# wienkers/marEx

Measured on AMD Instinct MI355X. Metric: Mcells*timesteps/s, shifting_baseline + hobday_extreme p95 (validation+anomaly+thresholds+mask), higher is better.
Workload: dtype f32

## Files before the change

marex_amd/csrc/marex_shifting.hip:

```cpp
#include "marex_common.hip.h"
#include "marex_tails.hip.h"
#include <numeric>
#include <utility>

template <int D, int SCAP, bool SEXACT, int WCAP, bool RREG>
__global__ void __launch_bounds__(256)
k_shifting(const float* __restrict__ x, long T, long C, const int4* __restrict__ year_plan, int n_cal, int W,
           int S_rt, int write_clim, const float* __restrict__ edges, int nb, long T_out, float* __restrict__ out,
           unsigned short* __restrict__ bins, unsigned char* __restrict__ mask, int* __restrict__ invalid_count,
           int ncb, int nchunks, const int* __restrict__ skip) {
    extern __shared__ float lds[];
    float* ring = lds;
    float rr[RREG ? D : 1][RREG ? WCAP : 1];
    const int npad = WCAP - W;
    int4* lplan = reinterpret_cast<int4*>(lds + (RREG ? (size_t)0 : (size_t)D * WCAP * 256));
    float* e = reinterpret_cast<float*>(lplan + (size_t)n_cal * D);

    int cb, chunk;
    if (!xcd_swizzle(blockIdx.x, ncb, nchunks, cb, chunk)) return;
    if (D == 4 && skip && skip[chunk]) return;
    const int tid = threadIdx.x;
    const long c = (long)cb * 256 + tid;
    const bool active = c < C;
    const int S = SEXACT ? SCAP : S_rt;
// ... 343 lines not shown
            int4 e[4];
            for (int i = 0; i < 4; ++i)
                e[i] = (d0 + i < NDOY) ? year_plan[(size_t)y * NDOY + d0 + i] : make_int4(-1, -1, -1, 0);
            int m = 0;
            while (m < 4 && e[m].x >= 0) ++m;
            if (fplan) {
                const int yn = y + 1 < n_cal ? y + 1 : n_cal - 1;
                const int tbw = year_plan[(size_t)yn * NDOY + (chunk >> 2) * 16].x;
                fplan[((size_t)y * 92 + chunk) * 2] = make_int4(e[0].x, e[0].y, m, e[0].z);
                fplan[((size_t)y * 92 + chunk) * 2 + 1] = make_int4(e[1].z, e[2].z, e[3].z, tbw);
            }
            for (int i = m; i < 4; ++i) ok = ok && e[i].x < 0;
            for (int i = 1; i < m; ++i) {
                ok = ok && e[i].x == e[0].x + i;
                if (e[0].y >= 0)
                    ok = ok && e[i].y == e[0].y + i && e[i].z >= 0;
                else
                    ok = ok && e[i].y < 0;
            }
            if (m > 0 && e[0].y >= 0) ok = ok && e[0].z >= 0;
        }
        if (!ok) atomicAnd(&s_ok[chunk], 0);
    }
    __syncthreads();
    if (chunk < 92 && lplan && reg_S > 0) {
        const int H = reg_S / 2, NPAIR = (reg_S + 3) / 2, NROWS = wpb * ((reg_S + 4 * wpb - 1 + wpb - 1) / wpb);
        const int d0 = chunk * 4, blk16 = (chunk / wpb) * wpb * 4;
        int D1 = 0, D2 = 0, D3 = 0;
        if (lean_bins && d0 + 3 < NDOY)
            for (int y2 = 0; y2 < n_cal; ++y2) {
                const int z0 = year_plan[(size_t)y2 * NDOY + d0].z, z1 = year_plan[(size_t)y2 * NDOY + d0 + 1].z;
                const int z2 = year_plan[(size_t)y2 * NDOY + d0 + 2].z, z3 = year_plan[(size_t)y2 * NDOY + d0 + 3].z;
                if (z0 >= 0 && z1 >= 0 && z2 >= 0 && z3 >= 0) {
                    D1 = z1 - z0;
                    D2 = z2 - z0;
                    D3 = z3 - z0;
                    break;
                }
            }
        for (int yy = sub - 1; yy <= n_cal; yy += CLASSIFY_SPLIT) {
            int flags = 0, tbv = -1, pos = 0;
            long long xoff = 0, ooff = 0;
            if (yy + 1 >= 0 && yy + 1 < n_cal) {
                const int tbn = year_plan[(size_t)(yy + 1) * NDOY + blk16].x;
                if (tbn >= H && (long)tbn - H + NROWS <= T) {
                    flags |= 4;
                    xoff = (long long)(tbn - H) * C * 4;
                }
            }
            if (yy >= 0 && yy < n_cal) {
                int4 e[4];
                for (int i = 0; i < 4; ++i) e[i] = (d0 + i < NDOY) ? year_plan[(size_t)yy * NDOY + d0 + i] : make_int4(-1, -1, -1, 0);
                tbv = year_plan[(size_t)yy * NDOY + blk16].x;
                int reg = d0 + 3 < NDOY && e[0].x >= 0 && e[1].x >= 0 && e[2].x >= 0 && e[3].x >= 0;
                reg = reg && tbv >= H && (long)tbv - H + NROWS <= T && e[0].x == tbv + 4 * (chunk % wpb);
                reg = reg && e[0].x - H >= 0 && (long)e[0].x - H + 2 * NPAIR <= T;
                for (int i = 1; i < 4; ++i) reg = reg && e[i].x == e[0].x + i && ((e[0].y >= 0) == (e[i].y >= 0));
                if (e[0].y >= 0) {
                    flags |= 2;
                    ooff = (long long)e[0].y * C * 4;
                    if (lean_bins) {
                        pos = e[0].z;
                        reg = reg && pos >= 0 && e[1].z == pos + D1 && e[2].z == pos + D2 && e[3].z == pos + D3;
                        for (int i = 1; i < 4; ++i) reg = reg && e[i].y == e[0].y + i;
                    } else {
                        pos = e[0].z - doy_start[d0];
                        reg = reg && pos >= 0 && pos < TAIL_MAX_BUCKET;
                        for (int i = 1; i < 4; ++i) reg = reg && e[i].y == e[0].y + i && e[i].z - doy_start[d0 + i] == pos;
                    }
                }
                if (reg) flags |= 1;
            }
            int4* r = lplan + ((size_t)(yy + 1) * LEAN_CHUNKS + chunk) * 2;
            r[0] = make_int4(flags, tbv, (int)(unsigned)(xoff & 0xFFFFFFFFll), (int)(unsigned)((unsigned long long)xoff >> 32));
            r[1] = make_int4((int)(unsigned)(ooff & 0xFFFFFFFFll), (int)(unsigned)((unsigned long long)ooff >> 32), pos, 0);
            if (yy < 0 && lean_bins) r[1] = make_int4(0, D1, D2, D3);
            if (chunk + 4 >= 92 && chunk + 4 < (92 + wpb - 1) / wpb * wpb) {
                r[8] = make_int4(flags & 4, tbv, (int)(unsigned)(xoff & 0xFFFFFFFFll), (int)(unsigned)((unsigned long long)xoff >> 32));
                r[9] = make_int4(0, 0, 0, 0);
            }
        }
    }
    if (t < 92) info[t] = s_ok[t] && s_edges_ok;
}

#define SHIFT_LIST 15
struct TailOut {
    uint4* lists;
    unsigned* aux;
    const int* doy_start;
    int nper;
    unsigned long long* dbg;
};

template <int W, bool TAILS, int S = 21>
__global__ void __launch_bounds__(256)
k_shift_fast(const float* __restrict__ x, long T, long C, const int4* __restrict__ fplan, int n_cal,
             const int* __restrict__ info, int write_clim, const float* __restrict__ edges, int nb, long T_out, float* __restrict__ out, unsigned short* __restrict__ bins, unsigned char* __restrict__ mask,
             int* __restrict__ invalid_count, int ncg, int nblk, TailOut tails) {
    int cg, bc;
    if (!xcd_swizzle(blockIdx.x, ncg, nblk, cg, bc)) return;
    const int wave = __builtin_amdgcn_readfirstlane((int)(threadIdx.x >> 6));
    const int lane = (int)(threadIdx.x & 63);
    const int chunk = bc * 4 + wave;
    static_assert((S & 1) == 1 && S >= 5 && S <= 25, "k_shift_fast: odd smoothing widths 5..25");
    constexpr int H = S / 2, NPAIR = (S + 3) / 2, NST = S + 15, RPW = (NST + 3) / 4;
    constexpr int NSTAGE = TAILS ? 1 : 2;
    constexpr int NROWS = NST;
    __shared__ float stage[NSTAGE][NROWS * 64];
    __shared__ unsigned newkeys[TAILS ? 4 : 1][2][TAILS ? SHIFT_LIST : 1][64];
    const bool mine = chunk < 92 && info[chunk] != 0;
    const int d0 = mine ? chunk * 4 : 0;
    const int4* prec = fplan + (size_t)chunk * 2;
    constexpr size_t YREC = 92 * 2;
    const long c = (long)cg * 64 + lane;
    const bool active = c < C;
    const unsigned cidx = active ? (unsigned)c : (unsigned)(C - 1);
    const bool do_bins = bins != nullptr && !TAILS;
    const unsigned voff = cidx * 4u;
    const int rowb = (int)(C * 4);
    const unsigned bin_lane = (((cidx >> 4) - (unsigned)(cg * 4)) * (unsigned)T_out * 16u + (cidx & 15u)) * 2u;
    const rsrc_t rbins = make_rsrc(do_bins ? bins + (size_t)(cg * 4) * (size_t)T_out * 16 : nullptr);

    float e_first = 0.f, e_delta = 1.f, inv_width = 1.f, e_last = 0.f;
    if (do_bins || TAILS) {
        e_first = edges[1];
        e_delta = edges[2] - edges[1];
        e_last = edges[nb];
        inv_width = (float)(nb - 1) / (e_last - e_first);
    }
    constexpr float Sf = (float)S;
    const float yS = 1.0f / Sf;
    const float Wf = (float)W;
    const float yW = 1.0f / Wf;
    const float nbm1f = (float)(nb - 1);
    const float c0 = (1.0f - e_first * inv_width) - 0.0078125f;
    const float qnan = nan_f();

    if (chunk == 0 && mine && mask && active) mask[c] = finite_f(x[c]) ? 1 : 0;
    auto stage_ok = [&](int tb) { return tb >= H && (long)tb - H + NROWS <= T; };
    auto stage_load = [&](int tb, float (&nx)[RPW]) {
        const rsrc_t rs = make_rsrc(x + (size_t)(tb - H + RPW * wave) * C);
#pragma unroll
        for (int k = 0; k < RPW; ++k)
            if (4 * RPW == NST || RPW * wave + k < NST) nx[k] = ldb_f32(rs, voff, k * rowb);
    };
    auto stage_store = [&](int buf, const float (&nx)[RPW]) {
#pragma unroll
        for (int k = 0; k < RPW; ++k)
            if (4 * RPW == NST || RPW * wave + k < NST) stage[buf & (NSTAGE - 1)][(RPW * wave + k) * 64 + lane] = nx[k];
    };
    int tb_cur = fplan[(size_t)(bc * 4) * 2].x;
    int tb_n1 = prec[1].w;
    {
        float nx[RPW];
        if (stage_ok(tb_cur)) {
            stage_load(tb_cur, nx);
            stage_store(0, nx);
        }
        __syncthreads();
    }

    v2f rA[W + 2], rB[W + 2];
#pragma unroll
    for (int j = 0; j < W + 2; ++j) rA[j] = rB[j] = splat2(qnan);
    int n_invalid = 0;
    unsigned t_cntA = 0, t_cntB = 0, t_ovfA = 0, t_ovfB = 0;
    int t_slot = 0, t_list = 0;
    int t_ds0 = 0, t_ds1 = 0, t_ds2 = 0, t_ds3 = 0;
    if (TAILS && mine) {
        t_ds0 = tails.doy_start[d0];
        t_ds1 = tails.doy_start[d0 + 1 < NDOY ? d0 + 1 : NDOY - 1];
        t_ds2 = tails.doy_start[d0 + 2 < NDOY ? d0 + 2 : NDOY - 1];
        t_ds3 = tails.doy_start[d0 + 3 < NDOY ? d0 + 3 : NDOY - 1];
    }
    auto tails_flush = [&]() {
        const tl_out_rsrc_t rl = tl_out_make_rsrc(tails.lists + (size_t)d0 * tails.nper * 2 * (size_t)C);
        const unsigned lvoff = cidx * 16u;
#pragma unroll
        for (int pr = 0; pr < 2; ++pr) {
            unsigned v[16];
#pragma unroll
            for (int u = 0; u < 16; ++u) v[u] = (u < SHIFT_LIST && u < t_slot) ? newkeys[wave][pr][u][lane] : 0u;
            sort16_desc(v);
#pragma unroll
            for (int h = 0; h < 2; ++h) {
                const int di = 2 * pr + h;
                if (d0 + di < NDOY) {
#pragma unroll
                    for (int jj = 0; jj < 2; ++jj) {
                        unsigned w[4];
#pragma unroll
                        for (int i = 0; i < 4; ++i) {
                            const unsigned a = v[8 * jj + 2 * i], b = v[8 * jj + 2 * i + 1];
                            w[i] = h == 0 ? ((a & 0xFFFFu) | (b << 16)) : ((a >> 16) | (b & 0xFFFF0000u));
                        }
                        const int li = __builtin_amdgcn_readfirstlane((di * tails.nper + t_list) * 2 + jj);
                        tl_out_store(rl, lvoff, (unsigned)li * (unsigned)C * 16u, w);
                    }
                }
            }
        }
        ++t_list;
        t_slot = 0;
    };

    int4 nA = prec[0], nB = prec[1];
    auto one_year = [&](int y, auto Jc) {
        constexpr int J = decltype(Jc)::value;
        const int4 pA = nA, pB = nB;
        const int tb = tb_cur;
        float nx[RPW];
        const bool stage_next = y + 1 < n_cal && stage_ok(tb_n1);
        if (stage_next) stage_load(tb_n1, nx);
        v2f smA = splat2(qnan), smB = splat2(qnan);
        v2f xp[NPAIR];
        const bool staged = mine && pA.z > 0 && stage_ok(tb) && pA.x == tb + 4 * wave;
        if (staged) {
            const float* st = &stage[y & (NSTAGE - 1)][(4 * wave) * 64 + lane];
#pragma unroll
            for (int m = 0; m < NPAIR; ++m) {
                xp[m].x = st[(2 * m) * 64];
                xp[m].y = st[(2 * m + 1) * 64];
            }
        }
        if (TAILS) {
            asm volatile("s_waitcnt lgkmcnt(0)\n\ts_barrier" ::: "memory");
        }
        else asm volatile("" ::: "memory");
        {
            const int y1 = y + 1 < n_cal ? y + 1 : n_cal - 1;
            nA = prec[(size_t)y1 * YREC];
            nB = prec[(size_t)y1 * YREC + 1];
            tb_cur = tb_n1;
            tb_n1 = nB.w;
        }
        if (mine && pA.z > 0) {
            const long r0 = (long)pA.x - H;
            const bool edge = r0 < 0 || r0 + 2 * NPAIR > T;
            if (staged) {
            } else if (!edge) {
                const rsrc_t rx = make_rsrc(x + (size_t)r0 * C);
#pragma unroll
                for (int m = 0; m < NPAIR; ++m) {
                    xp[m].x = ldb_f32(rx, voff, (2 * m) * rowb);
                    xp[m].y = ldb_f32(rx, voff, (2 * m + 1) * rowb);
                }
            } else {
#pragma unroll
                for (int m = 0; m < NPAIR; ++m) {
                    long ra = r0 + 2 * m, rb = ra + 1;
                    ra = ra < 0 ? 0 : (ra > T - 1 ? T - 1 : ra);
                    rb = rb < 0 ? 0 : (rb > T - 1 ? T - 1 : rb);
                    xp[m].x = ldb_f32(make_rsrc(x + (size_t)ra * C), voff, 0);
                    xp[m].y = ldb_f32(make_rsrc(x + (size_t)rb * C), voff, 0);
                }
            }
            v2f accA = (v2f){xp[0].x, -0.0f};
#pragma unroll
// ... 58 lines not shown
                                ++n[i];
                            }
                    }
                    if (!(climA.x == climA.x)) climA.x = acc[0] / (float)n[0];
                    if (!(climA.y == climA.y)) climA.y = acc[1] / (float)n[1];
                    if (!(climB.x == climB.x)) climB.x = acc[2] / (float)n[2];
                    if (!(climB.y == climB.y)) climB.y = acc[3] / (float)n[3];
                }
                const v2f aA = xcA - climA, aB = xcB - climB;
                const rsrc_t ro = make_rsrc(out + (size_t)pA.y * C);
                stb_f32(ro, voff, 0, write_clim ? climA.x : aA.x);
                if (has1) stb_f32(ro, voff, rowb, write_clim ? climA.y : aA.y);
                if (has2) stb_f32(ro, voff, 2 * rowb, write_clim ? climB.x : aB.x);
                if (has3) stb_f32(ro, voff, 3 * rowb, write_clim ? climB.y : aB.y);
                if (do_bins || TAILS) {
                    auto digit2 = [&](v2f a, int& k0, int& k1) {
                        const v2f f = __builtin_elementwise_fma(a, splat2(inv_width), splat2(c0));
                        v2f t;
                        t.x = __builtin_amdgcn_fmed3f(__builtin_floorf(f.x), 0.0f, nbm1f);
                        t.y = __builtin_amdgcn_fmed3f(__builtin_floorf(f.y), 0.0f, nbm1f);
                        const v2f phi = t * splat2(e_delta);
                        const v2f ehi = splat2(e_first) + phi;
                        k0 = (int)t.x + (a.x >= ehi.x ? 1 : 0);
                        k1 = (int)t.y + (a.y >= ehi.y ? 1 : 0);
                        if (!TAILS) {
                            k0 = (a.x == a.x) ? k0 : nb;
                            k1 = (a.y == a.y) ? k1 : nb;
                        }
                    };
                    int k0, k1, k2, k3;
                    digit2(aA, k0, k1);
                    digit2(aB, k2, k3);
                    if (TAILS) {
                        const float l1 = has1 ? e_last : -__builtin_inff(), l2 = has2 ? e_last : -__builtin_inff(),
                                    l3 = has3 ? e_last : -__builtin_inff();
                        const bool v0 = aA.x < e_last, v1 = aA.y < l1, v2 = aB.x < l2, v3 = aB.y < l3;
                        const unsigned b0 = 128u + (unsigned)(pA.w - t_ds0), b1 = 128u + (unsigned)(pB.x - t_ds1);
                        const unsigned b2 = 128u + (unsigned)(pB.y - t_ds2), b3 = 128u + (unsigned)(pB.z - t_ds3);
                        const unsigned q0 = v0 ? ((unsigned)k0 << TAIL_POS_BITS) + b0 : 0u, q1 = v1 ? ((unsigned)k1 << TAIL_POS_BITS) + b1 : 0u;
                        const unsigned q2 = v2 ? ((unsigned)k2 << TAIL_POS_BITS) + b2 : 0u, q3 = v3 ? ((unsigned)k3 << TAIL_POS_BITS) + b3 : 0u;
                        newkeys[wave][0][t_slot][lane] = q0 | (q1 << 16);
                        newkeys[wave][1][t_slot][lane] = q2 | (q3 << 16);
                        t_cntA += (v0 ? 1u : 0u) + (v1 ? 0x10000u : 0u);
                        t_cntB += (v2 ? 1u : 0u) + (v3 ? 0x10000u : 0u);
                        const float mx = fmaxf(fmaxf(aA.x, has1 ? aA.y : aA.x), fmaxf(has2 ? aB.x : aA.x, has3 ? aB.y : aA.x));
                        if (__builtin_amdgcn_ballot_w64(mx >= e_last) != 0) {
                            unsigned s0 = t_ovfA & 0xFFFFu, s1 = t_ovfA >> 16, s2 = t_ovfB & 0xFFFFu, s3 = t_ovfB >> 16;
                            if (aA.x >= e_last) s0 = tail_ovf_add(s0, (unsigned)(pA.w - t_ds0));
                            if (has1 && aA.y >= e_last) s1 = tail_ovf_add(s1, (unsigned)(pB.x - t_ds1));
                            if (has2 && aB.x >= e_last) s2 = tail_ovf_add(s2, (unsigned)(pB.y - t_ds2));
                            if (has3 && aB.y >= e_last) s3 = tail_ovf_add(s3, (unsigned)(pB.z - t_ds3));
                            t_ovfA = s0 | (s1 << 16);
                            t_ovfB = s2 | (s3 << 16);
                        }
                        ++t_slot;
                    } else {
                        stb_u16(rbins, bin_lane, pA.w * 32, k0);
                        if (has1) stb_u16(rbins, bin_lane, pB.x * 32, k1);
                        if (has2) stb_u16(rbins, bin_lane, pB.y * 32, k2);
                        if (has3) stb_u16(rbins, bin_lane, pB.z * 32, k3);
                    }
                }
            }
        }
        rA[J + W] = smA;
        rB[J + W] = smB;
        if (stage_next) stage_store((y + 1) & 1, nx);
        __syncthreads();
    };
    for (int y = 0; y < n_cal; y += 2) {
        one_year(y, std::integral_constant<int, 0>{});
        if (TAILS && t_slot == SHIFT_LIST) tails_flush();
        if (y + 1 < n_cal) one_year(y + 1, std::integral_constant<int, 1>{});
        if (TAILS && t_slot == SHIFT_LIST) tails_flush();
#pragma unroll
        for (int j = 0; j < W; ++j) {
            rA[j] = rA[j + 2];
            rB[j] = rB[j + 2];
        }
    }
    if (TAILS && mine) {
        if (t_slot > 0) tails_flush();
        while (t_list < tails.nper) tails_flush();
        if (active) {
            const unsigned cn[4] = {t_cntA & 0xFFFFu, t_cntA >> 16, t_cntB & 0xFFFFu, t_cntB >> 16};
            const unsigned ov[4] = {t_ovfA & 0xFFFFu, t_ovfA >> 16, t_ovfB & 0xFFFFu, t_ovfB >> 16};
#pragma unroll
            for (int di = 0; di < 4; ++di)
                if (d0 + di < NDOY) tails.aux[(size_t)(d0 + di) * C + c] = tail_aux_word(cn[di], ov[di]);
        }
    }
    if (invalid_count && active && n_invalid) atomicAdd(&invalid_count[c], n_invalid);
}

template <typename F, int... Is>
__device__ __forceinline__ void unroll_steps_impl(F& f, std::integer_sequence<int, Is...>) {
    (f(std::integral_constant<int, Is>{}), ...);
}
template <int N, typename F>
__device__ __forceinline__ void unroll_steps(F&& f) {
    unroll_steps_impl(f, std::make_integer_sequence<int, N>{});
}

#define LR_REG 1
#define LR_OUT 2
#define LR_STAGE_NEXT 4

template <int W, int S, int NWV, bool BINS>
__global__ void __launch_bounds__(64 * NWV, 16 / NWV)
k_shift_lean(const float* __restrict__ x, int T, int C, const int4* __restrict__ fplan, const int4* __restrict__ lplan, int n_cal,
             const int* __restrict__ info, const float* __restrict__ edges, int nb, float* __restrict__ out,
             unsigned char* __restrict__ mask, int* __restrict__ invalid_count, int ncg, int nblk, TailOut tails,
             unsigned short* __restrict__ bins, long T_out) {
    int cg, bc;
    if (!xcd_swizzle(blockIdx.x, ncg, nblk, cg, bc)) return;
    const int wave = __builtin_amdgcn_readfirstlane((int)(threadIdx.x >> 6));
    const int lane = (int)(threadIdx.x & 63);
    const int chunk = bc * NWV + wave;
    static_assert((S & 1) == 1 && S >= 5 && S <= 25, "k_shift_lean: odd smoothing widths 5..25");
    static_assert(NWV == 4 || NWV == 8, "k_shift_lean: 4 or 8 waves");
    constexpr int H = S / 2, NPAIR = (S + 3) / 2, NST = S + 4 * NWV - 1, RPW = (NST + NWV - 1) / NWV;
    constexpr int NROWS = NWV * RPW;
    __shared__ float stage[NROWS * 64];
    __shared__ unsigned newkeys[BINS ? 1 : NWV][2][BINS ? 1 : SHIFT_LIST][64];
    const bool mine = chunk < 92 && info[chunk] != 0;
    const int d0 = mine ? chunk * 4 : 0;
    const int c = cg * 64 + lane;
    const bool active = c < C;
    const unsigned cidx = active ? (unsigned)c : (unsigned)(C - 1);
    const unsigned voff = cidx * 4u;
    const int rowb = C * 4;
    const float e_first = edges[1], e_delta = edges[2] - edges[1], e_last = edges[nb];
    const float inv_width = (float)(nb - 1) / (e_last - e_first);
    constexpr float Sf = (float)S;
    const float yS = 1.0f / Sf;
    const float Wf = (float)W;
    const float yW = 1.0f / Wf;
    const float nbm1f = (float)(nb - 1);
    const float c0 = (1.0f - e_first * inv_width) - 0.0078125f;
    const float qnan = nan_f();
    if (chunk == 0 && mine && mask && active) mask[c] = finite_f(x[c]) ? 1 : 0;
    const unsigned bin_lane = (((cidx >> 4) - (unsigned)(cg * 4)) * (unsigned)T_out * 16u + (cidx & 15u)) * 2u;
    const rsrc_t rbins = make_rsrc(BINS ? bins + (size_t)(cg * 4) * (size_t)T_out * 16 : nullptr);
    int bD1 = 0, bD2 = 0, bD3 = 0;

    typedef __attribute__((address_space(3))) float lds_f32;
    const int c4 = cg * 64 + (lane & 15) * 4;
    const unsigned dma_voff4 = (unsigned)(lane >> 4) * (unsigned)rowb + (unsigned)(c4 + 4 <= C ? c4 : C - 4) * 4u;
    const unsigned dma_lds = (unsigned)__builtin_amdgcn_readfirstlane((int)(unsigned)(size_t)(lds_f32*)&stage[(RPW * wave) * 64]);
    const char* xw = reinterpret_cast<const char*>(x) + (size_t)(RPW * wave) * (size_t)C * 4;
    auto dma_rows = [&](int lo, int hi) __attribute__((always_inline)) {
        const unsigned long long off = ((unsigned long long)(unsigned)hi << 32) | (unsigned)lo;
        DmaRows<RPW>::issue(tl_out_make_rsrc(xw + off), dma_voff4, voff, dma_lds, 256u, 0u, (unsigned)rowb);
    };
    constexpr int LSTRIDE = LEAN_CHUNKS * 2;
    const int4* lr_next = lplan + (size_t)chunk * 2;
    {
        const int4 pre = lr_next[0];
        if (BINS) {
            const int4 preB = lr_next[1];
            bD1 = preB.y;
            bD2 = preB.z;
            bD3 = preB.w;
        }
        if (pre.x & LR_STAGE_NEXT) {
            dma_rows(pre.z, pre.w);
            asm volatile("s_waitcnt vmcnt(0)" ::: "memory");
        }
        asm volatile("s_barrier" ::: "memory");
        lr_next += LSTRIDE;
    }
    int4 nA = lr_next[0], nB = lr_next[1];
    lr_next += LSTRIDE;

    constexpr int U = W >= 13 ? 3 : 2;
    v2f hA[W + U], hB[W + U];
#pragma unroll
    for (int j = 0; j < W + U; ++j) hA[j] = hB[j] = splat2(qnan);
    int n_invalid = 0;
    unsigned t_cntA = 0, t_cntB = 0, t_ovfA = 0, t_ovfB = 0;
    int t_slot = 0, t_list = 0;
    auto tails_flush = [&]() __attribute__((always_inline)) {
        const tl_out_rsrc_t rl = tl_out_make_rsrc(tails.lists + (size_t)d0 * tails.nper * 2 * (size_t)C);
        const unsigned lvoff = cidx * 16u;
#pragma unroll
        for (int pr = 0; pr < 2; ++pr) {
            unsigned v[16];
#pragma unroll
            for (int u = 0; u < 16; ++u) v[u] = (u < SHIFT_LIST && u < t_slot) ? newkeys[wave][pr][u][lane] : 0u;
            sort16_desc(v);
#pragma unroll
            for (int h = 0; h < 2; ++h) {
                const int di = 2 * pr + h;
                if (d0 + di < NDOY) {
#pragma unroll
                    for (int jj = 0; jj < 2; ++jj) {
                        unsigned w[4];
#pragma unroll
                        for (int i = 0; i < 4; ++i) {
                            const unsigned a = v[8 * jj + 2 * i], b = v[8 * jj + 2 * i + 1];
                            w[i] = h == 0 ? ((a & 0xFFFFu) | (b << 16)) : ((a >> 16) | (b & 0xFFFF0000u));
                        }
                        const int li = __builtin_amdgcn_readfirstlane((di * tails.nper + t_list) * 2 + jj);
                        if (active) tl_out_store(rl, lvoff, (unsigned)li * (unsigned)C * 16u, w);
                    }
                }
            }
        }
        ++t_list;
        t_slot = 0;
    };

    auto mid = [&](const int4& cA) __attribute__((always_inline)) {
        asm volatile("s_waitcnt lgkmcnt(0)\n\ts_barrier" ::: "memory");
        if (cA.x & LR_STAGE_NEXT) dma_rows(cA.z, cA.w);
        nA = lr_next[0];
        nB = lr_next[1];
        lr_next += LSTRIDE;
    };
    constexpr int NH0 = (NPAIR + 1) / 2, NH1 = NPAIR - NH0;
    static_assert(NH0 >= 2, "the second chain starts in the first half");
    v2f xh[NH0];
    v2f accA = splat2(0.f), accB = splat2(0.f);
    float xc0 = 0.f, xc1 = 0.f, xc2 = 0.f, xc3 = 0.f;
    auto load_half = [&](auto Pc, int how, int ts) __attribute__((always_inline)) {
        constexpr int P = decltype(Pc)::value, M0 = P ? NH0 : 0, MN = P ? NH1 : NH0;
        if (how == 0) {
            const float* st = &stage[(4 * wave) * 64 + lane];
#pragma unroll
            for (int m = 0; m < MN; ++m) {
                xh[m].x = st[(2 * (M0 + m)) * 64];
                xh[m].y = st[(2 * (M0 + m) + 1) * 64];
            }
        } else if (how == 1) {
            const rsrc_t rx = make_rsrc(x + (size_t)(ts - H) * (size_t)C);
#pragma unroll
            for (int m = 0; m < MN; ++m) {
                xh[m].x = ldb_f32(rx, voff, (2 * (M0 + m)) * rowb);
                xh[m].y = ldb_f32(rx, voff, (2 * (M0 + m) + 1) * rowb);
            }
        } else {
#pragma unroll
            for (int m = 0; m < MN; ++m) {
                int ra = ts - H + 2 * (M0 + m), rb = ra + 1;
                ra = ra < 0 ? 0 : (ra > T - 1 ? T - 1 : ra);
                rb = rb < 0 ? 0 : (rb > T - 1 ? T - 1 : rb);
                xh[m].x = ldb_f32(make_rsrc(x + (size_t)ra * (size_t)C), voff, 0);
                xh[m].y = ldb_f32(make_rsrc(x + (size_t)rb * (size_t)C), voff, 0);
            }
        }
    };
    auto half = [&](auto Pc) __attribute__((always_inline)) {
        constexpr int P = decltype(Pc)::value, M0 = P ? NH0 : 0, M1 = P ? NPAIR : NH0;
        if constexpr (S == 21) {
#define PK_LO(acc, src) "v_pk_add_f32 %" #acc ", %" #acc ", %" #src " op_sel_hi:[1,0]\n\t"
#define PK_HI(acc, src) "v_pk_add_f32 %" #acc ", %" #acc ", %" #src " op_sel:[0,1] op_sel_hi:[1,1]\n\t"
#define PK_BOTH(src) PK_LO(0, src) PK_LO(1, src) PK_HI(0, src) PK_HI(1, src)
            if (P == 0) {
                accA = (v2f){xh[0].x, -0.0f};
                accB = (v2f){xh[1].x, -0.0f};
                asm(PK_HI(0, 2) PK_LO(0, 3) PK_HI(0, 3) PK_HI(1, 3) PK_BOTH(4) PK_BOTH(5) PK_BOTH(6) PK_BOTH(7)
                    : "+v"(accA), "+v"(accB)
                    : "v"(xh[0]), "v"(xh[1]), "v"(xh[2]), "v"(xh[3]), "v"(xh[4]), "v"(xh[5]));
                xc0 = xh[5].x;
                xc1 = xh[5].y;
// ... 211 lines not shown
            if (has2) n_invalid += finite_f(xcB.x) ? 0 : 1; else smB.x = qnan;
            if (has3) n_invalid += finite_f(xcB.y) ? 0 : 1; else smB.y = qnan;
            asm volatile("s_waitcnt vmcnt(0)" ::: "memory");
            if (pA.y >= 0) {
                v2f aA, aB;
                anomaly(Jc, xcA, xcB, aA, aB);
                const rsrc_t ro = make_rsrc(out + (size_t)pA.y * (size_t)C);
                if (active) {
                    stb_f32(ro, voff, 0, aA.x);
                    if (has1) stb_f32(ro, voff, rowb, aA.y);
                    if (has2) stb_f32(ro, voff, 2 * rowb, aB.x);
                    if (has3) stb_f32(ro, voff, 3 * rowb, aB.y);
                }
                int k0, k1, k2, k3;
                digit2(aA, k0, k1);
                digit2(aB, k2, k3);
                if constexpr (BINS) {
                    if (active) {
                        stb_u16(rbins, bin_lane, pA.w * 32, (aA.x == aA.x) ? k0 : nb);
                        if (has1) stb_u16(rbins, bin_lane, pB.x * 32, (aA.y == aA.y) ? k1 : nb);
                        if (has2) stb_u16(rbins, bin_lane, pB.y * 32, (aB.x == aB.x) ? k2 : nb);
                        if (has3) stb_u16(rbins, bin_lane, pB.z * 32, (aB.y == aB.y) ? k3 : nb);
                    }
                } else {
                const float l1 = has1 ? e_last : -__builtin_inff(), l2 = has2 ? e_last : -__builtin_inff(),
                            l3 = has3 ? e_last : -__builtin_inff();
                const bool v0 = aA.x < e_last, v1 = aA.y < l1, v2 = aB.x < l2, v3 = aB.y < l3;
                const int ds0 = tails.doy_start[d0], ds1 = tails.doy_start[d0 + 1 < NDOY ? d0 + 1 : NDOY - 1];
                const int ds2 = tails.doy_start[d0 + 2 < NDOY ? d0 + 2 : NDOY - 1], ds3 = tails.doy_start[d0 + 3 < NDOY ? d0 + 3 : NDOY - 1];
                const unsigned p0 = (unsigned)(pA.w - ds0), p1 = (unsigned)(pB.x - ds1), p2 = (unsigned)(pB.y - ds2), p3 = (unsigned)(pB.z - ds3);
                const unsigned q0 = v0 ? ((unsigned)k0 << TAIL_POS_BITS) + 128u + p0 : 0u, q1 = v1 ? ((unsigned)k1 << TAIL_POS_BITS) + 128u + p1 : 0u;
                const unsigned q2 = v2 ? ((unsigned)k2 << TAIL_POS_BITS) + 128u + p2 : 0u, q3 = v3 ? ((unsigned)k3 << TAIL_POS_BITS) + 128u + p3 : 0u;
                newkeys[wave][0][t_slot][lane] = q0 | (q1 << 16);
                newkeys[wave][1][t_slot][lane] = q2 | (q3 << 16);
                t_cntA += (v0 ? 1u : 0u) + (v1 ? 0x10000u : 0u);
                t_cntB += (v2 ? 1u : 0u) + (v3 ? 0x10000u : 0u);
                const float mx = fmaxf(fmaxf(aA.x, has1 ? aA.y : aA.x), fmaxf(has2 ? aB.x : aA.x, has3 ? aB.y : aA.x));
                if (__builtin_amdgcn_ballot_w64(mx >= e_last) != 0) {
                    unsigned s0 = t_ovfA & 0xFFFFu, s1 = t_ovfA >> 16, s2 = t_ovfB & 0xFFFFu, s3 = t_ovfB >> 16;
                    if (aA.x >= e_last) s0 = tail_ovf_add(s0, p0);
                    if (has1 && aA.y >= e_last) s1 = tail_ovf_add(s1, p1);
                    if (has2 && aB.x >= e_last) s2 = tail_ovf_add(s2, p2);
                    if (has3 && aB.y >= e_last) s3 = tail_ovf_add(s3, p3);
                    t_ovfA = s0 | (s1 << 16);
                    t_ovfB = s2 | (s3 << 16);
                }
                ++t_slot;
                }
            }
        } else {
            mid(cA);
            asm volatile("s_waitcnt vmcnt(0)" ::: "memory");
        }
        hA[J + W] = smA;
        hB[J + W] = smB;
    };

#define MAREX_LEAN_YEAR(J, yy)                                                                                  \
    {                                                                                                           \
        const int4 cA = nA, cB = nB;                                                                            \
        if (mine && (cA.x & LR_REG)) {                                                                          \
            lean_year(std::integral_constant<int, J>{}, cA, cB);                                                \
        } else {                                                                                                \
            general_year(std::integral_constant<int, J>{}, yy, cA);                                             \
        }                                                                                                       \
        asm volatile("s_barrier" ::: "memory");  \
        if (!BINS && t_slot == SHIFT_LIST) tails_flush();                                                       \
    }
    for (int y = 0; y < n_cal; y += U) {
        MAREX_LEAN_YEAR(0, y)
        if constexpr (U > 1) if (y + 1 < n_cal) MAREX_LEAN_YEAR(1, y + 1)
        if constexpr (U > 2) if (y + 2 < n_cal) MAREX_LEAN_YEAR(2, y + 2)
        if constexpr (U > 3) if (y + 3 < n_cal) MAREX_LEAN_YEAR(3, y + 3)
#pragma unroll
        for (int j = 0; j < W; ++j) {
            hA[j] = hA[j + U];
            hB[j] = hB[j + U];
        }
    }
#undef MAREX_LEAN_YEAR
    if (mine && !BINS) {
        if (t_slot > 0) tails_flush();
        while (t_list < tails.nper) tails_flush();
        if (active) {
            const unsigned cn[4] = {t_cntA & 0xFFFFu, t_cntA >> 16, t_cntB & 0xFFFFu, t_cntB >> 16};
            const unsigned ov[4] = {t_ovfA & 0xFFFFu, t_ovfA >> 16, t_ovfB & 0xFFFFu, t_ovfB >> 16};
#pragma unroll
            for (int di = 0; di < 4; ++di)
                if (d0 + di < NDOY) tails.aux[(size_t)(d0 + di) * (size_t)C + c] = tail_aux_word(cn[di], ov[di]);
        }
    }
    if (invalid_count && active && n_invalid) atomicAdd(&invalid_count[c], n_invalid);
}

static bool lean_instance(int W, int S) { return S == 21 && (W == 15 || W == 5); }

struct ShiftArgs {
    const float* x;
    int64_t T, C;
    const int4* year_plan;
    const int4* fplan;
    int n_cal;
    int W, S, write_clim;
    const float* edges;
    int nb;
    int64_t T_out;
    float* out;
    uint16_t* bins;
    uint8_t* mask;
    int32_t* invalid_count;
    const int* skip;
    TailOut tails;
    bool lean = false;
    const int4* lplan = nullptr;
    int lean_waves = 4;
};

template <int D, int SCAP, bool SEXACT, int WCAP, bool RREG>
static int launch_shifting(marex_ctx* ctx, const ShiftArgs& a) {
    const int ncb = (int)((a.C + 255) / 256);
    const int nchunks = (NDOY + D - 1) / D;
    const size_t lds = ((RREG ? (size_t)0 : (size_t)D * WCAP * 256) + (a.bins ? (size_t)a.nb + 1 : 0)) * sizeof(float) + (size_t)a.n_cal * D * 16;
    if (lds > 80 * 1024) return fail(ctx, -4, "marex_shifting_baseline_f32: window_year_baseline=%d needs more than 80 KiB of LDS", a.W);
    auto kern = k_shifting<D, SCAP, SEXACT, WCAP, RREG>;
    if (lds > 48 * 1024)
        HIP_TRY(ctx, hipFuncSetAttribute((const void*)kern, hipFuncAttributeMaxDynamicSharedMemorySize, (int)lds));
    hipLaunchKernelGGL(kern, dim3(xcd_grid(ncb, nchunks)), dim3(256), lds, ctx->stream, a.x, (long)a.T, (long)a.C,
                       a.year_plan, a.n_cal, a.W, a.S, a.write_clim, a.edges, a.nb, (long)a.T_out, a.out, a.bins,
                       a.mask, a.invalid_count, ncb, nchunks, D == 4 ? a.skip : nullptr);
    HIP_TRY(ctx, hipGetLastError());
    return 0;
}

template <int W, int S = 21>
static void launch_shift_fast(marex_ctx* ctx, const ShiftArgs& a) {
    const int ncg = (int)((a.C + 63) / 64);
#define MAREX_SF_ARGS dim3(xcd_grid(ncg, 23)), dim3(256), 0, ctx->stream, a.x, (long)a.T, (long)a.C, a.fplan, a.n_cal, a.skip, a.write_clim, a.edges, a.nb, (long)a.T_out, a.out, a.bins, a.mask, a.invalid_count, ncg, 23, a.tails
    if (a.lean && (a.tails.lists || a.bins)) {
        if constexpr (S == 21 && (W == 15 || W == 5)) {
            if (a.tails.lists)
                hipLaunchKernelGGL((k_shift_lean<W, S, 4, false>), dim3(xcd_grid(ncg, 23)), dim3(256), 0, ctx->stream, a.x, (int)a.T, (int)a.C,
                                   a.fplan, a.lplan, a.n_cal, a.skip, a.edges, a.nb, a.out, a.mask, a.invalid_count, ncg, 23, a.tails,
                                   (unsigned short*)nullptr, (long)a.T_out);
            else
                hipLaunchKernelGGL((k_shift_lean<W, S, 4, true>), dim3(xcd_grid(ncg, 23)), dim3(256), 0, ctx->stream, a.x, (int)a.T, (int)a.C,
                                   a.fplan, a.lplan, a.n_cal, a.skip, a.edges, a.nb, a.out, a.mask, a.invalid_count, ncg, 23, a.tails,
                                   a.bins, (long)a.T_out);
        }
    } else if (a.tails.lists) {
        hipLaunchKernelGGL((k_shift_fast<W, true, S>), MAREX_SF_ARGS);
    } else {
        hipLaunchKernelGGL((k_shift_fast<W, false, S>), MAREX_SF_ARGS);
    }
#undef MAREX_SF_ARGS
}

template <int D, int WCAP, bool RREG>
static int dispatch_shifting_S(marex_ctx* ctx, const ShiftArgs& a) {
    if (a.S == 21) return launch_shifting<D, 21, true, WCAP, RREG>(ctx, a);
    return launch_shifting<D, 1, false, WCAP, RREG>(ctx, a);
}

static int shifting_impl(marex_ctx* ctx, const char* who, const float* x, int64_t T, int64_t C, const int32_t* year_plan,
                         int n_cal_years, int W, int S, int write_clim, const float* edges, int nb, int64_t T_out, float* out,
                         uint16_t* bins, uint8_t* mask, int32_t* invalid_count, TailOut tails, bool* all_fast_possible) {
    if (!ctx) return -1;
    if (!x || !year_plan || !out || T <= 0 || C <= 0 || n_cal_years <= 0)
        return fail(ctx, -1, "%s: null pointer or empty shape", who);
// ... 116 lines not shown
```

marex_amd/csrc/marex_tails.hip:

```cpp
#include "marex_common.hip.h"
#include "marex_tails.hip.h"

typedef __amdgpu_buffer_rsrc_t tl_rsrc_t;
__device__ __forceinline__ tl_rsrc_t tl_make_rsrc(const void* base) {
    return __builtin_amdgcn_make_buffer_rsrc(const_cast<void*>(base), 0, -1, 0x00020000);
}
__device__ __forceinline__ uint4 tl_load_chunk(tl_rsrc_t r, unsigned voff, unsigned soff) {
    typedef unsigned u4 __attribute__((ext_vector_type(4)));
    const u4 v = __builtin_amdgcn_raw_buffer_load_b128(r, (int)voff, (int)soff, 0);
    return make_uint4(v.x, v.y, v.z, v.w);
}
__device__ __forceinline__ unsigned pk_sub_sat_u16(unsigned a, unsigned b) {
    unsigned r;
    asm("v_pk_sub_u16 %0, %1, %2 clamp" : "=v"(r) : "v"(a), "v"(b));
    return r;
}
__device__ __forceinline__ unsigned pk_add_u16(unsigned a, unsigned b) {
    unsigned r;
    asm("v_pk_add_u16 %0, %1, %2" : "=v"(r) : "v"(a), "v"(b));
    return r;
}
__device__ __forceinline__ unsigned pk_sub_u16(unsigned a, unsigned b) {
    unsigned r;
    asm("v_pk_sub_u16 %0, %1, %2" : "=v"(r) : "v"(a), "v"(b));
// ... 746 lines not shown
            if (pass >= pass_limit) {
                if (!resolved) {
                    thr[(size_t)d * C + cell] = nan_f();
                    atomicAdd(&stats->n_unresolved, 1u);
                }
                break;
            }
            if (lo) {
                B0 = clamp_base(tried_lo - TT_STEP);
                tried_lo = B0;
            } else {
                B0 = clamp_base(tried_hi + TT_STEP);
                tried_hi = B0;
            }
            BW = nb - B0 < TT_BW ? nb - B0 : TT_BW;
            excursion = true;
            rebuild(d);
            tot_s[ci] = prefix();
            hint = -1;
            ++n_pass;
        }
        if (dd + 1 < ndays) {
            const int imin = s_iumin[dpar], imax = s_iumax[dpar];
            if (imax >= 0) {
                const int span = imax - imin + 1;
                const bool near_edge = imin - B0 < TT_MARGIN || (B0 + BW - 1) - imax < TT_MARGIN;
                if (excursion || near_edge) {
                    const int want = clamp_base(span <= TT_BW - 2 * TT_MARGIN ? imin - (TT_BW - span) / 2 : imin - TT_MARGIN);
                    if (want != B0) {
                        B0 = want;
                        BW = nb - B0 < TT_BW ? nb - B0 : TT_BW;
                        need_rebuild = true;
                    }
                }
            }
        }
    }
    for (int sft = 32; sft > 0; sft >>= 1) {
        const unsigned a = __shfl_down(kmin, sft, 64), b = __shfl_down(kmax, sft, 64);
        kmin = a < kmin ? a : kmin;
        kmax = b > kmax ? b : kmax;
        nlow += __shfl_down(nlow, sft, 64);
        nhigh += __shfl_down(nhigh, sft, 64);
    }
    if ((t & 63) == 0) {
        if (kmin != 0xFFFFFFFFu) atomicMin(&stats->min_key, kmin);
        if (kmax != 0u) atomicMax(&stats->max_key, kmax);
        if (nlow) atomicAdd(&stats->n_too_low, nlow);
        if (nhigh) atomicAdd(&stats->n_too_high, nhigh);
    }
    if (dbg && t == 0) {
        atomicAdd(&dbg[0], n_rebuild);
        atomicAdd(&dbg[2], n_pass);
        atomicAdd(&dbg[3], (unsigned long long)ndays);
    }
}

template <int NSC>
__global__ void __launch_bounds__(64)
k_thr_cells(const uint4* __restrict__ lists, const unsigned* __restrict__ aux, int NPER, int nch, const float* __restrict__ anom,
            long C, long c0, long c1, int nblk, const float* __restrict__ centres, int nb, double q, int wd, float lower_bound,
            float upper_bound, float* __restrict__ thr, marex_thr_stats* __restrict__ stats, unsigned long long* __restrict__ dbg) {
    extern __shared__ uint4 ring[];
    const int lane = (int)threadIdx.x;
    const long cell_raw = c0 + (long)blockIdx.x * 64 + lane;
    const bool valid = cell_raw < c1;
    const long cell = valid ? cell_raw : c1 - 1;
    const int d_begin = (int)blockIdx.y * NDOY / nblk, d_end = ((int)blockIdx.y + 1) * NDOY / nblk;
    const bool land = !(anom[cell] == anom[cell]);
    if (__builtin_amdgcn_ballot_w64(valid && !land) == 0) {
        if (valid)
            for (int d = d_begin; d < d_end; ++d) thr[(size_t)d * C + cell] = nan_f();
        return;
    }
    const int pd = wd / 2, nslot = (wd * NPER + 3) & ~3;
    uint4* mine = ring + lane;
    for (int k = wd * NPER; k < nslot; ++k) mine[k * 64] = make_uint4(0, 0, 0, 0);
    const unsigned voff = (unsigned)cell * 16u, chunk_row = (unsigned)C * 16u;
    const size_t day_stride = (size_t)NPER * nch * (size_t)C;
    auto wrap = [](int d) { return d < 0 ? d + NDOY : (d >= NDOY ? d - NDOY : d); };
    auto cnt_of = [&](int day) { return (int)(aux[(size_t)day * C + cell] & 0x3FFu); };
    auto load_day = [&](int day, int k) {
        const tl_rsrc_t r = tl_make_rsrc(lists + (size_t)day * day_stride);
        for (int p = 0; p < NPER; ++p) mine[((k % wd) * NPER + p) * 64] = tl_load_chunk(r, voff, (unsigned)(nch * p) * chunk_row);
    };
    int tot = 0;
    for (int o = 0; o < wd; ++o) {
        const int day = wrap(d_begin - pd + o);
        load_day(day, o);
        tot += cnt_of(day);
    }
    uint4 cache[NSC > 0 ? NSC : 1];
    auto count_ring = [&](int b) {
        const unsigned lim = ((unsigned)(b + 1) << TAIL_POS_BITS) - 1u, lim_rep = lim | (lim << 16);
        unsigned acc0 = 0, acc1 = 0;
        if (NSC > 0) {
#pragma unroll
            for (int k = 0; k < NSC; ++k) {
                acc0 += pk_min1_u16(pk_sub_sat_u16(cache[k].x, lim_rep)) + pk_min1_u16(pk_sub_sat_u16(cache[k].z, lim_rep));
                acc1 += pk_min1_u16(pk_sub_sat_u16(cache[k].y, lim_rep)) + pk_min1_u16(pk_sub_sat_u16(cache[k].w, lim_rep));
            }
        } else
        for (int k = 0; k < nslot; k += 4) {
            const uint4 c[4] = {mine[k * 64], mine[(k + 1) * 64], mine[(k + 2) * 64], mine[(k + 3) * 64]};
#pragma unroll
            for (int u = 0; u < 4; ++u) {
                acc0 += pk_min1_u16(pk_sub_sat_u16(c[u].x, lim_rep)) + pk_min1_u16(pk_sub_sat_u16(c[u].z, lim_rep));
                acc1 += pk_min1_u16(pk_sub_sat_u16(c[u].y, lim_rep)) + pk_min1_u16(pk_sub_sat_u16(c[u].w, lim_rep));
            }
        }
        const unsigned acc = acc0 + acc1;
        return (int)((acc & 0xFFFFu) + (acc >> 16));
    };
    auto count_exact = [&](int d, int b) {
        const unsigned lim = ((unsigned)(b + 1) << TAIL_POS_BITS) - 1u, lim_rep = lim | (lim << 16);
        int n = 0;
        for (int o = -pd; o <= pd; ++o) {
            const tl_rsrc_t r = tl_make_rsrc(lists + (size_t)wrap(d + o) * day_stride);
            for (int p = 0; p < NPER; ++p)
                for (int jj = 0; jj < nch; ++jj) n += tl_count_above(tl_load_chunk(r, voff, (unsigned)(nch * p + jj) * chunk_row), lim_rep);
        }
        return n;
    };
    unsigned kmin = 0xFFFFFFFFu, kmax = 0u, nlow = 0u, nhigh = 0u;
    unsigned long long n_exact = 0;
    for (int d = d_begin; d < d_end; ++d) {
        if (d > d_begin) {
            const int din = wrap(d + pd), dout = wrap(d - pd - 1);
            load_day(din, d - d_begin - 1);
            tot += cnt_of(din) - cnt_of(dout);
        }
        if (NSC > 0) {
#pragma unroll
            for (int k = 0; k < NSC; ++k) cache[k] = mine[k * 64];
        }
        unsigned kfull = 0, khead = 0, ktail = 0xFFFFu;
        int nlists = 0;
        for (int k = 0; k < nslot; k += 4) {
            const uint4 c[4] = {mine[k * 64], mine[(k + 1) * 64], mine[(k + 2) * 64], mine[(k + 3) * 64]};
#pragma unroll
            for (int u = 0; u < 4; ++u) {
                kfull = c[u].w > kfull ? c[u].w : kfull;
                const unsigned head = c[u].x & 0xFFFFu;
                khead = head > khead ? head : khead;
                ktail = (head != 0u && head < ktail) ? head : ktail;
                nlists += head != 0u ? 1 : 0;
            }
        }
        kfull >>= 16;
        float t32 = nan_f();
        if (tot > 0) {
            const double qpos = q * (double)tot;
            int lo = -1, hi = nb - 1, n_lo = tot, n_hi = 0;
            if (khead != 0u && (double)tot > qpos) {
                const int bh = (int)(khead >> TAIL_POS_BITS) - 1;
                hi = bh < hi ? bh : hi;
            }
            bool lo_exact = true;
            if (nlists > 0 && (double)(tot - nlists) <= qpos) {
                const int bt = (int)(ktail >> TAIL_POS_BITS) - 2;
                if (bt > lo && bt < hi) {
                    lo = bt;
                    n_lo = nlists;
                    lo_exact = false;
                }
            }
            while (__builtin_amdgcn_ballot_w64(hi - lo > 1) != 0) {
                const bool go = hi - lo > 1;
                const int mid = go ? (lo + hi) >> 1 : hi;
                int n = count_ring(mid + 1);
                const unsigned first = (unsigned)(mid + 2) << TAIL_POS_BITS;
                bool exact = !(first <= kfull);
                bool f = (double)(tot - n) <= qpos;
                if (__builtin_amdgcn_ballot_w64(go && !f && !exact) != 0) {
                    const int ne = count_exact(d, mid + 1);
                    if (go && !f && !exact) {
                        n = ne;
                        exact = true;
                        f = (double)(tot - n) <= qpos;
                        ++n_exact;
                    }
                }
                if (go) {
                    if (f) {
                        lo = mid;
                        n_lo = n;
                        lo_exact = exact;
                    } else {
                        hi = mid;
                        n_hi = n;
                    }
                }
            }
            const int iu = hi;
            if (__builtin_amdgcn_ballot_w64(iu > 0 && !lo_exact) != 0) {
                const int ne = count_exact(d, iu);
                if (iu > 0 && !lo_exact) {
                    n_lo = ne;
                    ++n_exact;
                }
            }
            const int il = iu > 0 ? iu - 1 : 0;
            const int cs_iu = tot - n_hi, cs_il = iu > 0 ? tot - n_lo : cs_iu;
            const int diff = cs_iu - cs_il;
            const double frac = diff > 0 ? (qpos - (double)cs_il) / (double)diff : 0.5;
            const float dc = centres[iu] - centres[il];
            const double prod = frac * (double)dc;
            t32 = (float)((double)centres[il] + prod);
            if (iu == 0) t32 = centres[0];
            if (valid && !land) {
                const unsigned key = ordered_key(t32);
                kmin = key < kmin ? key : kmin;
                kmax = key > kmax ? key : kmax;
// ... 96 lines not shown
            const long cost = ((blocks + slots - 1) / slots) * (d + wd);
            if (best < 0 || cost < best) best = cost, Dd = d;
        }
    }
    dim3 grid((unsigned)(tiles_x * tiles_y), (unsigned)((NDOY + Dd - 1) / Dd));
    unsigned long long* dbg = ctx_debug_counters(ctx);
    const uint4* tl = reinterpret_cast<const uint4*>(lists);
    const int pass_limit = ctx_opt(ctx, "THR_PASS_LIMIT", 2 * (nb / TT_STEP) + 9);
#define MAREX_TT_ARGS tl, aux, NPER, nch, anom, (long)C, ny, nx, row0, row1, tiles_x, Dd, centres, nb, q, wd, lower_bound, upper_bound, thr_doy_major, stats, dbg, pass_limit
#define MAREX_TT_LAUNCH(PP, TCC, NTT, ...)                                                                                           \
    do {                                                                                                                             \
        if (NPER <= 1)                                                                                                               \
            hipLaunchKernelGGL((k_thr_tails<PP, TCC, NTT, 1, ##__VA_ARGS__>), grid, dim3(NTT), 0, ctx->stream, MAREX_TT_ARGS);       \
        else if (NPER <= 2)                                                                                                          \
            hipLaunchKernelGGL((k_thr_tails<PP, TCC, NTT, 2, ##__VA_ARGS__>), grid, dim3(NTT), 0, ctx->stream, MAREX_TT_ARGS);       \
        else                                                  \
            hipLaunchKernelGGL((k_thr_tails<PP, TCC, NTT, 3, ##__VA_ARGS__>), grid, dim3(NTT), 0, ctx->stream, MAREX_TT_ARGS);       \
    } while (0)
    const bool lean = NPER == 6 && nch == 2 && big && p == 2 && ctx_opt(ctx, "THR_LEAN", 1) != 0;
    {
        LaunchTimer lt(ctx, MAREX_K_THRESHOLDS);
        if (lean && tall)
            hipLaunchKernelGGL((k_thr_tails<2, 30, 1024, 3, 34, 6, 2>), grid, dim3(1024), 0, ctx->stream, MAREX_TT_ARGS);
        else if (lean)
            hipLaunchKernelGGL((k_thr_tails<2, 32, 1024, 3, 32, 6, 2>), grid, dim3(1024), 0, ctx->stream, MAREX_TT_ARGS);
        else if (TR == 1)
            MAREX_TT_LAUNCH(0, 256, 256);
        else if (big && p == 1)
            MAREX_TT_LAUNCH(1, 32, 1024);
        else if (big && p == 2 && tall)
            MAREX_TT_LAUNCH(2, 30, 1024, 34);
        else if (big && p == 2)
            MAREX_TT_LAUNCH(2, 32, 1024);
        else if (big)
            MAREX_TT_LAUNCH(3, 32, 1024);
        else if (p == 1)
            MAREX_TT_LAUNCH(1, 16, 256);
        else if (p == 2)
            MAREX_TT_LAUNCH(2, 16, 256);
        else
            MAREX_TT_LAUNCH(3, 16, 256);
    }
#undef MAREX_TT_LAUNCH
#undef MAREX_TT_ARGS
    HIP_TRY(ctx, hipGetLastError());
    return 0;
}

template <bool RING>
__global__ void __launch_bounds__(64)
k_thr_pool(const uint4* __restrict__ lists, const unsigned* __restrict__ aux, int NPER, int nch, const float* __restrict__ anom,
           long C, long c0, long c1, int nblk, const int* __restrict__ pool, int K, const float* __restrict__ centres, int nb,
           double q, int wd, float lower_bound, float upper_bound, float* __restrict__ thr, marex_thr_stats* __restrict__ stats,
           unsigned long long* __restrict__ dbg) {
    extern __shared__ uint4 pool_smem[];
    const int lane = (int)threadIdx.x;
    const long cell = c0 + (long)blockIdx.x * 64 + lane;
    const bool valid = cell < c1;
    const int d_begin = (int)blockIdx.y * NDOY / nblk, d_end = ((int)blockIdx.y + 1) * NDOY / nblk;
    const bool land = valid ? !(anom[cell] == anom[cell]) : true;
    if (__builtin_amdgcn_ballot_w64(!land) == 0) {
        if (valid)
            for (int d = d_begin; d < d_end; ++d) thr[(size_t)d * C + cell] = nan_f();
        return;
    }
    int* mem = reinterpret_cast<int*>(pool_smem) + lane;
    for (int m = 0; m < K; ++m) mem[m * 64] = land ? -1 : pool[(size_t)m * C + cell];
    uint4* ring = pool_smem + K * 16 + lane;
    const int pd = wd / 2, per_day = K * NPER, nslot = (wd * per_day + 3) & ~3;
    if (RING)
        for (int k = wd * per_day; k < nslot; ++k) ring[k * 64] = make_uint4(0, 0, 0, 0);
    const unsigned chunk_row = (unsigned)C * 16u;
    const size_t day_stride = (size_t)NPER * nch * (size_t)C;
    auto wrap = [](int d) { return d < 0 ? d + NDOY : (d >= NDOY ? d - NDOY : d); };
    auto cnt_of = [&](int day) {
        int n = 0;
        for (int m = 0; m < K; ++m) {
            const int j = mem[m * 64];
            if (j >= 0) n += (int)(aux[(size_t)day * C + j] & 0x3FFu);
        }
        return n;
    };
    auto global_first = [&](int day, int j, int p) {
        return tl_load_chunk(tl_make_rsrc(lists + (size_t)day * day_stride), (unsigned)j * 16u, (unsigned)(nch * p) * chunk_row);
    };
    auto load_day = [&](int day, int k) {
        if (!RING) return;
        for (int m = 0; m < K; ++m) {
            const int j = mem[m * 64];
            for (int p = 0; p < NPER; ++p) {
                const uint4 ch = j >= 0 ? global_first(day, j, p) : make_uint4(0, 0, 0, 0);
                ring[((k % wd) * per_day + m * NPER + p) * 64] = ch;
            }
        }
    };
    auto first_chunk = [&](int d, int i, int m, int p) {
        if (RING) return ring[(i * per_day + m * NPER + p) * 64];
        const int j = mem[m * 64];
        return j >= 0 ? global_first(wrap(d - pd + i), j, p) : make_uint4(0, 0, 0, 0);
    };
    int tot = 0;
    for (int o = 0; o < wd; ++o) {
        const int day = wrap(d_begin - pd + o);
        load_day(day, o);
        tot += cnt_of(day);
    }
    auto count_first = [&](int d, int b, int& sat) {
        const unsigned lim = ((unsigned)(b + 1) << TAIL_POS_BITS) - 1u, lim_rep = lim | (lim << 16);
        unsigned acc0 = 0, acc1 = 0, accl = 0;
        if (RING) {
            for (int k = 0; k < nslot; k += 4) {
                const uint4 c[4] = {ring[k * 64], ring[(k + 1) * 64], ring[(k + 2) * 64], ring[(k + 3) * 64]};
#pragma unroll
                for (int u = 0; u < 4; ++u) {
                    acc0 += pk_min1_u16(pk_sub_sat_u16(c[u].x, lim_rep)) + pk_min1_u16(pk_sub_sat_u16(c[u].z, lim_rep));
                    acc1 += pk_min1_u16(pk_sub_sat_u16(c[u].y, lim_rep));
                    accl += pk_min1_u16(pk_sub_sat_u16(c[u].w, lim_rep));
                }
            }
        } else
        for (int i = 0; i < wd; ++i)
            for (int m = 0; m < K; ++m)
                for (int p = 0; p < NPER; ++p) {
                    const uint4 c = first_chunk(d, i, m, p);
                    acc0 += pk_min1_u16(pk_sub_sat_u16(c.x, lim_rep)) + pk_min1_u16(pk_sub_sat_u16(c.z, lim_rep));
                    acc1 += pk_min1_u16(pk_sub_sat_u16(c.y, lim_rep));
                    accl += pk_min1_u16(pk_sub_sat_u16(c.w, lim_rep));
                }
        sat = (int)(accl >> 16);
        const unsigned acc = acc0 + acc1 + accl;
        return (int)((acc & 0xFFFFu) + (acc >> 16));
    };
    auto count_behind = [&](int d, int b, bool want) {
        const unsigned lim = ((unsigned)(b + 1) << TAIL_POS_BITS) - 1u, lim_rep = lim | (lim << 16);
        const int s0 = (d - d_begin) % wd;
        int n = 0;
        for (int i = 0; i < wd; ++i) {
            const int o = RING ? (i - s0 + wd) % wd : i;
            const tl_rsrc_t r = tl_make_rsrc(lists + (size_t)wrap(d - pd + o) * day_stride);
            for (int m = 0; m < K; ++m) {
                const int j = mem[m * 64];
                if (j < 0 || !want) continue;
                for (int p = 0; p < NPER; ++p) {
                    const uint4 c = first_chunk(d, i, m, p);
                    if ((c.w >> 16) <= lim) continue;
                    for (int jj = 1; jj < nch; ++jj) n += tl_count_above(tl_load_chunk(r, (unsigned)j * 16u, (unsigned)(nch * p + jj) * chunk_row), lim_rep);
                }
            }
        }
        return n;
    };
    unsigned kmin = 0xFFFFFFFFu, kmax = 0u, nlow = 0u, nhigh = 0u;
    unsigned long long n_exact = 0;
    for (int d = d_begin; d < d_end; ++d) {
        if (d > d_begin) {
            const int din = wrap(d + pd), dout = wrap(d - pd - 1);
            load_day(din, d - d_begin - 1);
            tot += cnt_of(din) - cnt_of(dout);
        }
        unsigned khead = 0, ktail = 0xFFFFu;
        int nlists = 0;
        auto see_head = [&](unsigned first_pair) {
            const unsigned head = first_pair & 0xFFFFu;
            khead = head > khead ? head : khead;
            ktail = (head != 0u && head < ktail) ? head : ktail;
            nlists += head != 0u ? 1 : 0;
        };
// ... 441 lines not shown
```

Measured before the change: 335,100.

## Skip flushing empty tail-key lists and defer zero fills to the end

The shifting kernels now skip the sort-and-store flush for a tail list when no lane in the wave gained new keys since the last flush. They record skipped list indices and write zeros for them only at the end, and only if some lane in the wave has a nonzero count. The tail consumers mask first-chunk loads by the per-day count and skip deeper chunk contributions using a header flag. This removes sort and store work for empty lists but adds ballots, extra aux reads and a dependency on the first-chunk header encoding.

```diff
diff --git a/marex_amd/csrc/marex_shifting.hip b/marex_amd/csrc/marex_shifting.hip
--- a/marex_amd/csrc/marex_shifting.hip
+++ b/marex_amd/csrc/marex_shifting.hip
@@ -449,6 +449,31 @@
         }
     }
     if (t < 92) info[t] = s_ok[t] && s_edges_ok;
+}
+
+__device__ __forceinline__ bool tails_list_has_keys(bool active, unsigned cntA, unsigned cntB, unsigned& seen) {
+    const unsigned sum = cntA + cntB;
+    const bool lane_has = sum != seen;
+    seen = sum;
+    return __builtin_amdgcn_ballot_w64(active && lane_has) != 0;
+}
+template <typename Rsrc>
+__device__ __forceinline__ void tails_fill_skipped(Rsrc rl, unsigned lvoff, bool store, const unsigned (&cn)[4], int d0, int nper, long C,
+                                                   unsigned skipped) {
+    const bool alive = (cn[0] | cn[1] | cn[2] | cn[3]) != 0u;
+    const unsigned sk = (unsigned)__builtin_amdgcn_readfirstlane((int)skipped);
+    if (sk == 0u || __builtin_amdgcn_ballot_w64(store && alive) == 0) return;
+    const unsigned zero[4] = {0u, 0u, 0u, 0u};
+    for (int p = 0; p < nper; ++p) {
+        if (((sk >> p) & 1u) == 0u) continue;
+        for (int di = 0; di < 4; ++di) {
+            if (d0 + di >= NDOY) break;
+            for (int jj = 0; jj < 2; ++jj) {
+                const int li = __builtin_amdgcn_readfirstlane((di * nper + p) * 2 + jj);
+                if (store) tl_out_store(rl, lvoff, (unsigned)li * (unsigned)C * 16u, zero);
+            }
+        }
+    }
 }
 
 #define SHIFT_LIST 15
@@ -541,7 +566,14 @@
         t_ds2 = tails.doy_start[d0 + 2 < NDOY ? d0 + 2 : NDOY - 1];
         t_ds3 = tails.doy_start[d0 + 3 < NDOY ? d0 + 3 : NDOY - 1];
     }
+    unsigned t_seen = 0, t_skipped = 0;
     auto tails_flush = [&]() {
+        if (!tails_list_has_keys(active, t_cntA, t_cntB, t_seen)) {
+            t_skipped |= 1u << t_list;
+            ++t_list;
+            t_slot = 0;
+            return;
+        }
         const tl_out_rsrc_t rl = tl_out_make_rsrc(tails.lists + (size_t)d0 * tails.nper * 2 * (size_t)C);
         const unsigned lvoff = cidx * 16u;
 #pragma unroll
@@ -766,8 +798,10 @@
     if (TAILS && mine) {
         if (t_slot > 0) tails_flush();
         while (t_list < tails.nper) tails_flush();
+        const unsigned cn[4] = {t_cntA & 0xFFFFu, t_cntA >> 16, t_cntB & 0xFFFFu, t_cntB >> 16};
+        tails_fill_skipped(tl_out_make_rsrc(tails.lists + (size_t)d0 * tails.nper * 2 * (size_t)C), cidx * 16u, active, cn, d0, tails.nper, C,
+                           t_skipped);
         if (active) {
-            const unsigned cn[4] = {t_cntA & 0xFFFFu, t_cntA >> 16, t_cntB & 0xFFFFu, t_cntB >> 16};
             const unsigned ov[4] = {t_ovfA & 0xFFFFu, t_ovfA >> 16, t_ovfB & 0xFFFFu, t_ovfB >> 16};
 #pragma unroll
             for (int di = 0; di < 4; ++di)
@@ -864,7 +898,14 @@
     int n_invalid = 0;
     unsigned t_cntA = 0, t_cntB = 0, t_ovfA = 0, t_ovfB = 0;
     int t_slot = 0, t_list = 0;
+    unsigned t_seen = 0, t_skipped = 0;
     auto tails_flush = [&]() __attribute__((always_inline)) {
+        if (!tails_list_has_keys(active, t_cntA, t_cntB, t_seen)) {
+            t_skipped |= 1u << t_list;
+            ++t_list;
+            t_slot = 0;
+            return;
+        }
         const tl_out_rsrc_t rl = tl_out_make_rsrc(tails.lists + (size_t)d0 * tails.nper * 2 * (size_t)C);
         const unsigned lvoff = cidx * 16u;
 #pragma unroll
@@ -1242,8 +1283,10 @@
     if (mine && !BINS) {
         if (t_slot > 0) tails_flush();
         while (t_list < tails.nper) tails_flush();
+        const unsigned cn[4] = {t_cntA & 0xFFFFu, t_cntA >> 16, t_cntB & 0xFFFFu, t_cntB >> 16};
+        tails_fill_skipped(tl_out_make_rsrc(tails.lists + (size_t)d0 * tails.nper * 2 * (size_t)C), cidx * 16u, active, cn, d0, tails.nper,
+                           (long)C, t_skipped);
         if (active) {
-            const unsigned cn[4] = {t_cntA & 0xFFFFu, t_cntA >> 16, t_cntB & 0xFFFFu, t_cntB >> 16};
             const unsigned ov[4] = {t_ovfA & 0xFFFFu, t_ovfA >> 16, t_ovfB & 0xFFFFu, t_ovfB >> 16};
 #pragma unroll
             for (int di = 0; di < 4; ++di)
diff --git a/marex_amd/csrc/marex_tails.hip b/marex_amd/csrc/marex_tails.hip
--- a/marex_amd/csrc/marex_tails.hip
+++ b/marex_amd/csrc/marex_tails.hip
@@ -852,14 +852,15 @@
     auto cnt_of = [&](int day) { return (int)(aux[(size_t)day * C + cell] & 0x3FFu); };
     auto load_day = [&](int day, int k) {
         const tl_rsrc_t r = tl_make_rsrc(lists + (size_t)day * day_stride);
-        for (int p = 0; p < NPER; ++p) mine[((k % wd) * NPER + p) * 64] = tl_load_chunk(r, voff, (unsigned)(nch * p) * chunk_row);
+        const int cnt = cnt_of(day);
+        for (int p = 0; p < NPER; ++p) {
+            const uint4 ch = tl_load_chunk(r, voff, (unsigned)(nch * p) * chunk_row);
+            mine[((k % wd) * NPER + p) * 64] = cnt > 0 ? ch : make_uint4(0, 0, 0, 0);
+        }
+        return cnt;
     };
     int tot = 0;
-    for (int o = 0; o < wd; ++o) {
-        const int day = wrap(d_begin - pd + o);
-        load_day(day, o);
-        tot += cnt_of(day);
-    }
+    for (int o = 0; o < wd; ++o) tot += load_day(wrap(d_begin - pd + o), o);
     uint4 cache[NSC > 0 ? NSC : 1];
     auto count_ring = [&](int b) {
         const unsigned lim = ((unsigned)(b + 1) << TAIL_POS_BITS) - 1u, lim_rep = lim | (lim << 16);
@@ -887,8 +888,16 @@
         int n = 0;
         for (int o = -pd; o <= pd; ++o) {
             const tl_rsrc_t r = tl_make_rsrc(lists + (size_t)wrap(d + o) * day_stride);
-            for (int p = 0; p < NPER; ++p)
-                for (int jj = 0; jj < nch; ++jj) n += tl_count_above(tl_load_chunk(r, voff, (unsigned)(nch * p + jj) * chunk_row), lim_rep);
+            const int k = (d - d_begin + o + pd) % wd;
+            for (int p = 0; p < NPER; ++p) {
+                const uint4 first = mine[(k * NPER + p) * 64];
+                const bool deeper = (first.w >> 16) != 0u;
+                n += tl_count_above(first, lim_rep);
+                for (int jj = 1; jj < nch; ++jj) {
+                    const int nk = tl_count_above(tl_load_chunk(r, voff, (unsigned)(nch * p + jj) * chunk_row), lim_rep);
+                    n += deeper ? nk : 0;
+                }
+            }
         }
         return n;
     };
@@ -897,8 +906,7 @@
     for (int d = d_begin; d < d_end; ++d) {
         if (d > d_begin) {
             const int din = wrap(d + pd), dout = wrap(d - pd - 1);
-            load_day(din, d - d_begin - 1);
-            tot += cnt_of(din) - cnt_of(dout);
+            tot += load_day(din, d - d_begin - 1) - cnt_of(dout);
         }
         if (NSC > 0) {
 #pragma unroll
@@ -1161,7 +1169,8 @@
         return n;
     };
     auto global_first = [&](int day, int j, int p) {
-        return tl_load_chunk(tl_make_rsrc(lists + (size_t)day * day_stride), (unsigned)j * 16u, (unsigned)(nch * p) * chunk_row);
+        const uint4 ch = tl_load_chunk(tl_make_rsrc(lists + (size_t)day * day_stride), (unsigned)j * 16u, (unsigned)(nch * p) * chunk_row);
+        return (aux[(size_t)day * C + j] & 0x3FFu) != 0u ? ch : make_uint4(0, 0, 0, 0);
     };
     auto load_day = [&](int day, int k) {
         if (!RING) return;
```

Result: no change. 338,100, median of 6 (+0.9%).
